# nilsfriess/ParMGMC

Measured on AMD Instinct MI355X. Metric: Gaussian samples/sec on 512^3 3D DMDA (7-pt Laplacian precision, red-black Gibbs sweep = 1 sorgibbs sample), higher is better.
Workload: dtype f64

## Files before the change

parmgmc_amd/csrc/kernels_grid.hip:

```cpp
#include <hip/hip_runtime.h>
#include <cstring>
#include <stdlib.h>
#include "pmg_kernels.h"
#define PMG_RNG_TU grid
#include "pmg_rng.hpp"

namespace {

typedef double d2 __attribute__((ext_vector_type(2)));

__device__ __forceinline__ d2 ld2(const double *p) { return *reinterpret_cast<const d2 *>(p); }

__device__ __forceinline__ d2 ld2_sys(const double *p)
{
  const unsigned long long a = __hip_atomic_load(reinterpret_cast<const unsigned long long *>(p), __ATOMIC_RELAXED, __HIP_MEMORY_SCOPE_SYSTEM);
  const unsigned long long b = __hip_atomic_load(reinterpret_cast<const unsigned long long *>(p) + 1, __ATOMIC_RELAXED, __HIP_MEMORY_SCOPE_SYSTEM);
  d2                       v;
  v.x = __longlong_as_double((long long)a);
  v.y = __longlong_as_double((long long)b);
  return v;
}
__device__ __forceinline__ void st2_sys(double *p, d2 v)
{
  __hip_atomic_store(reinterpret_cast<unsigned long long *>(p), (unsigned long long)__double_as_longlong(v.x), __ATOMIC_RELAXED, __HIP_MEMORY_SCOPE_SYSTEM);
  __hip_atomic_store(reinterpret_cast<unsigned long long *>(p) + 1, (unsigned long long)__double_as_longlong(v.y), __ATOMIC_RELAXED, __HIP_MEMORY_SCOPE_SYSTEM);
}

__device__ __forceinline__ const double *at_bytes(const double *base, uint32_t byte_off) { return reinterpret_cast<const double *>(reinterpret_cast<const char *>(base) + byte_off); }
__device__ __forceinline__ double       *at_bytes(double *base, uint32_t byte_off) { return reinterpret_cast<double *>(reinterpret_cast<char *>(base) + byte_off); }

__device__ __forceinline__ double uniform(double v)
{
  return __hiloint2double(__builtin_amdgcn_readfirstlane(__double2hiint(v)), __builtin_amdgcn_readfirstlane(__double2loint(v)));
}

template <bool PACKED>
__device__ __forceinline__ double table_at(const double (&a)[8], int idx)
{
  if (!PACKED) return uniform(a[idx]);
  double v = a[1];
  v        = idx == 2 ? a[2] : v;
  v        = idx == 3 ? a[3] : v;
  v        = idx == 4 ? a[4] : v;
  v        = idx == 5 ? a[5] : v;
  v        = idx == 6 ? a[6] : v;
  return v;
}

__device__ __forceinline__ void wave_wait_flag(const uint64_t *f, uint64_t v, unsigned *err, unsigned long long *spin_total)
{
  if (threadIdx.x == 0) {
    unsigned long long spins = 0;
    while (__hip_atomic_load(f, __ATOMIC_RELAXED, __HIP_MEMORY_SCOPE_SYSTEM) < v) {
      __builtin_amdgcn_s_sleep(8);
      ++spins;
      if ((spins & 0xFFFFu) == 0 && err && __hip_atomic_load(err, __ATOMIC_RELAXED, __HIP_MEMORY_SCOPE_SYSTEM)) break;
      if (spins > (1ull << 28)) {
        if (err) {
          err[1] = 0x10u;
          err[2] = (unsigned)v;
          err[3] = (unsigned)__hip_atomic_load(f, __ATOMIC_RELAXED, __HIP_MEMORY_SCOPE_SYSTEM);
          __hip_atomic_store(err, 1u, __ATOMIC_RELAXED, __HIP_MEMORY_SCOPE_SYSTEM);
        }
        break;
      }
    }
    if (spins && spin_total) atomicAdd(spin_total, spins);
  }
  __builtin_amdgcn_fence(__ATOMIC_ACQUIRE, "workgroup");
}

template <bool NOISY, bool OMEGA1, bool HALO, bool PACKED>
__device__ __forceinline__ void grid_color_sweep_body(const pmgk_grid_layout &L, const pmgk_grid_op &op, int c, int t, int j, int k, pmg::LogTabEntry *tab, pmg::LogTabEntry tab_entry, const pmgk_grid_halo &halo, const double *__restrict__ b_own, const double *__restrict__ y_other, double *__restrict__ y_own)
{
  const int kg = k + L.kz0;
  bool live = j < L.ny && 2 * t < L.sx && 4 * t + ((c + j + kg) & 1) < L.nx;
  if (NOISY) {
    if (!__builtin_amdgcn_ballot_w64(live)) return;
    t = live ? t : 0;
    if (PACKED) j = live ? j : 0;
  } else if (!live)
    return;
  const int p  = (c + j + kg) & 1;
  const int i0 = 4 * t + p, i1 = i0 + 2;
  const bool v1 = i1 < L.nx;

  const bool    hasS = j > 0, hasN = j < L.ny - 1, hasD = kg > 0, hasU = kg < L.nzg - 1;
  const double  h2 = op.h2;
  const int64_t  rowoff = (int64_t)(k + 1) * L.sp + (int64_t)j * L.sx;
  const uint32_t lo     = 16u * (uint32_t)t;
  const double  *yo_row = y_other + rowoff;
  const int    eo = p ? (2 * t + 2 < L.sx ? 2 : 1) : (t > 0 ? -1 : 0);
  const bool   hasW0 = i0 > 0, hasE0 = i0 < L.nx - 1, hasE1 = i1 < L.nx - 1;
  const int    nyz = PACKED ? (int)hasS + (int)hasN + (int)hasD + (int)hasU : min(j, 1) + min(L.ny - 1 - j, 1) + min(kg, 1) + min(L.nzg - 1 - kg, 1);
  const bool   two0 = hasW0 && hasE0, two1 = hasE1;
  const double idA = table_at<PACKED>(op.idiag, nyz + 1), idB = table_at<PACKED>(op.idiag, nyz + 2);
  const double sqA = NOISY ? table_at<PACKED>(op.sqrtdiag, nyz + 1) : 0.0, sqB = NOISY ? table_at<PACKED>(op.sqrtdiag, nyz + 2) : 0.0;
  double      *out_row = y_own + rowoff;
  d2     Vc = ld2(at_bytes(yo_row, lo));
  double ed = *at_bytes(yo_row, lo + 8u * (uint32_t)eo);
  d2     oS = ld2(at_bytes(yo_row - (hasS ? L.sx : 0), lo));
  d2     oN = ld2(at_bytes(yo_row + (hasN ? L.sx : 0), lo));
  const int64_t inplane = (int64_t)j * L.sx + 2 * t;
  d2      oD = (HALO && k == 0 && halo.glo) ? ld2_sys(halo.glo + inplane) : ld2(at_bytes(yo_row - (hasD ? L.sp : 0), lo));
  d2      oU = (HALO && k == L.nz - 1 && halo.ghi) ? ld2_sys(halo.ghi + inplane) : ld2(at_bytes(yo_row + (hasU ? L.sp : 0), lo));
#ifndef PMG_GRID_NO_NT
  d2     bb = __builtin_nontemporal_load(reinterpret_cast<const d2 *>(at_bytes(b_own + rowoff, lo)));
#else
  d2     bb = ld2(at_bytes(b_own + rowoff, lo));
#endif
  pmg::RngConsts K;
  if (NOISY) {
    __builtin_amdgcn_sched_barrier(0);
    K = pmg::load_sincos_consts();
    __builtin_amdgcn_sched_barrier(0);
  }

  double z0 = 0.0, z1 = 0.0;
  if (NOISY) {
    pmg::normal_pair_fill((uint32_t)t, (uint32_t)(j + (int64_t)L.ny * kg), (uint32_t)op.sweep, ((uint32_t)(op.sweep >> 32) & 0x7fffffffu) | ((uint32_t)c << 31), op.key0, op.key1, tab_entry, tab, (int)threadIdx.x, K, z0, z1);
    asm volatile("" : "+v"(Vc.x), "+v"(Vc.y), "+v"(ed), "+v"(oS.x), "+v"(oS.y), "+v"(oN.x), "+v"(oN.y), "+v"(oD.x), "+v"(oD.y), "+v"(oU.x), "+v"(oU.y), "+v"(bb.x), "+v"(bb.y) : "v"(z0), "v"(z1));
  }
  const double L0 = p ? Vc.x : ed, R0 = p ? Vc.y : Vc.x, L1 = R0, R1 = p ? ed : Vc.y;
  const double idg0 = two0 ? idB : idA, idg1 = two1 ? idB : idA;
  const double hS = hasS ? h2 : 0.0, hN = hasN ? h2 : 0.0, hD = hasD ? h2 : 0.0, hU = hasU ? h2 : 0.0;

  double w0 = bb.x, w1 = bb.y;
  if (NOISY) {
    const double sq0 = two0 ? sqB : sqA, sq1 = two1 ? sqB : sqA;
    w0 = z0 * sq0 + bb.x;
    w1 = z1 * sq1 + bb.y;
  }
  double s0 = w0, s1 = w1;
  s0 = s0 + hD * oD.x;
  s1 = s1 + hD * oD.y;
  s0 = s0 + hS * oS.x;
  s1 = s1 + hS * oS.y;
  s0 = s0 + (hasW0 ? h2 : 0.0) * L0;
  s1 = s1 + h2 * L1;
  s0 = s0 + (hasE0 ? h2 : 0.0) * R0;
  s1 = s1 + (hasE1 ? h2 : 0.0) * R1;
  s0 = s0 + hN * oN.x;
  s1 = s1 + hN * oN.y;
  s0 = s0 + hU * oU.x;
  s1 = s1 + hU * oU.y;

  double r0, r1;
  if (OMEGA1) {
    r0 = idg0 * s0;
    r1 = idg1 * s1;
  } else {
    const d2 yo2 = ld2(at_bytes(out_row, lo));
    r0           = op.one_minus_omega * yo2.x + idg0 * s0;
    r1           = op.one_minus_omega * yo2.y + idg1 * s1;
  }
  const d2 out = {r0, v1 ? r1 : 0.0};
  if (NOISY) {
    asm volatile("" ::"v"(out.x), "v"(out.y), "s"(out_row));
    if (!live) return;
  }
#ifndef PMG_GRID_NO_NT
  __builtin_nontemporal_store(out, reinterpret_cast<d2 *>(at_bytes(out_row, lo)));
#else
  *reinterpret_cast<d2 *>(at_bytes(out_row, lo)) = out;
#endif
  if (HALO) {
    if (k == 0 && halo.plo) st2_sys(halo.plo + inplane, out);
    if (k == L.nz - 1 && halo.phi) st2_sys(halo.phi + inplane, out);
  }
}

template <bool PACKED>
__device__ __forceinline__ void grid_thread_position(int nbx, int bandw, int ty, int &t, int &j)
{
  if (PACKED) {
    const int flat = ((int)blockIdx.x * 4 + ty) * 64 + (int)threadIdx.x;
    j              = flat / nbx;
    t              = flat - j * nbx;
  } else {
    const int bx = bandw > 0 ? (int)(blockIdx.x >> 3) : (int)blockIdx.x;
    const int jl = (int)blockIdx.y * 4 + ty;
    t            = bx * 64 + threadIdx.x;
    j            = bandw > 0 ? (jl < bandw ? (int)(blockIdx.x & 7u) * bandw + jl : 0x40000000) : jl;
  }
}

template <bool NOISY, bool OMEGA1, bool HALO, bool PACKED, bool TAIL>
__global__ __launch_bounds__(256) __attribute__((amdgpu_num_sgpr(96))) void grid_color_sweep_kernel(pmgk_grid_layout L, pmgk_grid_op op, int c, int nbx, int zmain, int bandw, int kbegin, int kstride, int kcount, int tmain, int tailw, pmgk_grid_halo halo, const double *__restrict__ b_own, const double *__restrict__ y_other, double *__restrict__ y_own)
{
  const int ty = __builtin_amdgcn_readfirstlane(threadIdx.y);
  __shared__ pmg::LogTabEntry s_logtab[NOISY ? 4 * PMG_LOGTAB_SIZE : 1];
  pmg::LogTabEntry           *tab = s_logtab + (NOISY ? ty * PMG_LOGTAB_SIZE : 0);
  pmg::LogTabEntry            tab_entry = {0.0, 0.0};
  if (NOISY) {
    const d2 e = ld2(reinterpret_cast<const double *>(pmg::g_logtab + threadIdx.x));
    tab_entry  = {e.x, e.y};
  }
  int                         t, j;
  const int                   zsplit = zmain > 0 ? zmain : kcount;
  if (TAIL && (int)blockIdx.z >= zsplit) {
    const int tb  = (int)blockIdx.x + (int)gridDim.x * ((int)blockIdx.y + (int)gridDim.y * ((int)blockIdx.z - zsplit));
    const bool compact = tailw == 1 && L.nx == 4 * tmain + 1 && (L.sx & 15) != 0;
    const int  slots   = compact ? (L.ny + 1) / 2 : L.ny * tailw;
    const int  per     = (slots + 255) / 256;
    const int  kz = tb / per, part = tb - kz * per;
    if (kz >= kcount) return;
    const int f = (part * 4 + ty) * 64 + (int)threadIdx.x, kt = kbegin + kz * kstride;
    if (compact) {
      j = 2 * f + ((c + kt + L.kz0) & 1);
      t = tmain;
    } else {
      j = f / tailw;
      t = tmain + f - j * tailw;
    }
    grid_color_sweep_body<NOISY, OMEGA1, false, true>(L, op, c, t, j, kt, tab, tab_entry, halo, b_own, y_other, y_own);
    return;
  }
  grid_thread_position<PACKED>(nbx, bandw, ty, t, j);

  int k = kbegin + (int)blockIdx.z * kstride;
  if (!HALO && !PACKED && zmain > 0) {
    const int xcd = (int)(blockIdx.x & 7u), extra = max(xcd - (8 - (L.ny - 8 * bandw)), 0);
    const int first = xcd * bandw + extra, nl = bandw + (xcd >= 8 - (L.ny - 8 * bandw) ? 1 : 0);
    const int w     = ((int)blockIdx.y + (int)gridDim.y * (int)blockIdx.z) * 4 + ty;
    if (nl <= 0) return;
    const int kz = w / nl;
    if (kz >= kcount) return;
    t = (int)(blockIdx.x >> 3) * 64 + (int)threadIdx.x;
    j = first + (w - kz * nl);
    k = kbegin + kz * kstride;
  }
  if (HALO && halo.full) {
    const int z = (int)blockIdx.z;
    k           = z == 0 ? 0 : (z == 1 ? L.nz - 1 : z - 1);
    const bool face_lo = k == 0, face_hi = k == L.nz - 1;
    if (face_lo && halo.wlo) wave_wait_flag(halo.wlo, halo.wval, halo.err, halo.spins);
    if (face_hi && halo.whi) wave_wait_flag(halo.whi, halo.wval, halo.err, halo.spins);
    grid_color_sweep_body<NOISY, OMEGA1, HALO, PACKED>(L, op, c, t, j, k, tab, tab_entry, halo, b_own, y_other, y_own);
    if (face_lo || face_hi) {
      asm volatile("s_waitcnt vmcnt(0)" ::: "memory");
      __builtin_amdgcn_fence(__ATOMIC_RELEASE, "workgroup");
      __syncthreads();
      if (threadIdx.x == 0 && threadIdx.y == 0) {
        const unsigned nface  = L.nz > 1 ? 2u : 1u;
        const unsigned expect = gridDim.x * gridDim.y * nface;
        if (atomicAdd(halo.counter, 1u) == expect - 1u) {
          *halo.counter = 0;
          if (halo.slo) __hip_atomic_store(halo.slo, halo.sval, __ATOMIC_RELAXED, __HIP_MEMORY_SCOPE_SYSTEM);
          if (halo.shi) __hip_atomic_store(halo.shi, halo.sval, __ATOMIC_RELAXED, __HIP_MEMORY_SCOPE_SYSTEM);
        }
      }
    }
    return;
  }
  grid_color_sweep_body<NOISY, OMEGA1, HALO, PACKED>(L, op, c, t, j, k, tab, tab_entry, halo, b_own, y_other, y_own);
}

__global__ void grid_to_cvec_kernel(pmgk_grid_layout L, const double *__restrict__ nat, double *__restrict__ cv)
{
  const int i = blockIdx.x * blockDim.x + threadIdx.x;
  const int j = blockIdx.y * blockDim.y + threadIdx.y;
  const int k = blockIdx.z;
  if (i >= L.nx || j >= L.ny) return;
  const int c = (i + j + k + L.kz0) & 1;
  cv[(int64_t)c * L.cs + (int64_t)(k + 1) * L.sp + (int64_t)j * L.sx + (i >> 1)] = nat[i + (int64_t)L.nx * (j + (int64_t)L.ny * k)];
}

__global__ void grid_from_cvec_kernel(pmgk_grid_layout L, const double *__restrict__ cv, double *__restrict__ nat)
{
  const int i = blockIdx.x * blockDim.x + threadIdx.x;
  const int j = blockIdx.y * blockDim.y + threadIdx.y;
  const int k = blockIdx.z;
  if (i >= L.nx || j >= L.ny) return;
  const int c = (i + j + k + L.kz0) & 1;
  nat[i + (int64_t)L.nx * (j + (int64_t)L.ny * k)] = cv[(int64_t)c * L.cs + (int64_t)(k + 1) * L.sp + (int64_t)j * L.sx + (i >> 1)];
}

struct residual_consts {
  double a, dA, dB, aS, aN, aD, aU;
};

__device__ __forceinline__ d2 residual_pair(const residual_consts &K, bool hasW0, bool hasE0, bool hasE1, bool v1, d2 oD, d2 oS, d2 oN, d2 oU, double L0, double R0, double L1, double R1, d2 yy, d2 bb)
{
  const double dg0 = (hasW0 && hasE0) ? K.dB : K.dA, dg1 = hasE1 ? K.dB : K.dA;
  double       s0 = 0.0, s1 = 0.0;
  s0 = s0 + K.aD * oD.x;
  s1 = s1 + K.aD * oD.y;
  s0 = s0 + K.aS * oS.x;
  s1 = s1 + K.aS * oS.y;
  s0 = s0 + (hasW0 ? K.a : 0.0) * L0;
  s1 = s1 + K.a * L1;
  s0 = s0 + dg0 * yy.x;
  s1 = s1 + dg1 * yy.y;
  s0 = s0 + (hasE0 ? K.a : 0.0) * R0;
  s1 = s1 + (hasE1 ? K.a : 0.0) * R1;
  s0 = s0 + K.aN * oN.x;
  s1 = s1 + K.aN * oN.y;
  s0 = s0 + K.aU * oU.x;
  s1 = s1 + K.aU * oU.y;
  const d2 out = {bb.x - s0, v1 ? bb.y - s1 : 0.0};
  return out;
}

template <bool PACKED>
__device__ __forceinline__ void grid_residual_values(const pmgk_grid_layout &L, const pmgk_grid_op &op, int t, int j, int k, const double *__restrict__ b, const double *__restrict__ y, int64_t &offa, int64_t &offb, d2 &outA, d2 &outB)
{
  const int      kg   = k + L.kz0;
  const int      ca   = (j + kg) & 1;
  const bool     hasS = j > 0, hasN = j < L.ny - 1, hasD = kg > 0, hasU = kg < L.nzg - 1;
  const int64_t  rowoff = (int64_t)(k + 1) * L.sp + (int64_t)j * L.sx;
  const uint32_t lo     = 16u * (uint32_t)t;
  offa = (int64_t)ca * L.cs + rowoff;
  offb = (int64_t)(1 - ca) * L.cs + rowoff;
  const double  *ya = y + offa, *yb = y + offb;
  const int64_t  dS = hasS ? L.sx : 0, dN = hasN ? L.sx : 0, dD = hasD ? L.sp : 0, dU = hasU ? L.sp : 0;
  const d2       Ya = ld2(at_bytes(ya, lo)), Yb = ld2(at_bytes(yb, lo));
  const double   edA = *at_bytes(yb, lo - (t > 0 ? 8u : 0u));
  const double   edB = *at_bytes(ya, lo + (2 * t + 2 < L.sx ? 16u : 8u));
  const int      nyz = (int)hasS + (int)hasN + (int)hasD + (int)hasU;
  residual_consts K;
  K.a  = -op.h2;
  K.dA = table_at<PACKED>(op.diag, nyz + 1);
  K.dB = table_at<PACKED>(op.diag, nyz + 2);
  K.aS = hasS ? K.a : 0.0;
  K.aN = hasN ? K.a : 0.0;
  K.aD = hasD ? K.a : 0.0;
  K.aU = hasU ? K.a : 0.0;
  const int i0 = 4 * t;
  outA = residual_pair(K, i0 > 0, i0 < L.nx - 1, i0 + 2 < L.nx - 1, i0 + 2 < L.nx, ld2(at_bytes(yb - dD, lo)), ld2(at_bytes(yb - dS, lo)), ld2(at_bytes(yb + dN, lo)), ld2(at_bytes(yb + dU, lo)), edA, Yb.x, Yb.x, Yb.y, Ya, ld2(at_bytes(b + offa, lo)));
  outB = d2{0.0, 0.0};
  if (i0 + 1 < L.nx)
    outB = residual_pair(K, true, i0 + 1 < L.nx - 1, i0 + 3 < L.nx - 1, i0 + 3 < L.nx, ld2(at_bytes(ya - dD, lo)), ld2(at_bytes(ya - dS, lo)), ld2(at_bytes(ya + dN, lo)), ld2(at_bytes(ya + dU, lo)), Ya.x, Ya.y, Ya.y, edB, Yb, ld2(at_bytes(b + offb, lo)));
}

template <bool PACKED>
__device__ __forceinline__ void grid_residual_body(const pmgk_grid_layout &L, const pmgk_grid_op &op, int t, int j, int k, const double *__restrict__ b, const double *__restrict__ y, double *__restrict__ r)
{
  if (j >= L.ny || 2 * t >= L.sx || 4 * t >= L.nx) return;
  int64_t offa, offb;
  d2      outA, outB;
  grid_residual_values<PACKED>(L, op, t, j, k, b, y, offa, offb, outA, outB);
  const uint32_t lo = 16u * (uint32_t)t;
  *reinterpret_cast<d2 *>(at_bytes(r + offa, lo)) = outA;
  if (4 * t + 1 < L.nx) *reinterpret_cast<d2 *>(at_bytes(r + offb, lo)) = outB;
}

__device__ __forceinline__ double lane_prev_d(double v)
{
  return __hiloint2double(__builtin_amdgcn_update_dpp(0, __double2hiint(v), 0x138, 0xf, 0xf, false), __builtin_amdgcn_update_dpp(0, __double2loint(v), 0x138, 0xf, 0xf, false));
}
__device__ __forceinline__ double lane_next_d(double v)
{
  return __hiloint2double(__builtin_amdgcn_update_dpp(0, __double2hiint(v), 0x130, 0xf, 0xf, false), __builtin_amdgcn_update_dpp(0, __double2loint(v), 0x130, 0xf, 0xf, false));
}

struct rr_acc {
  double s0, s1;
};
struct rr_thread {
  int      t, J0;
  uint32_t lo;
  bool     left, right0, right1;
  bool     eW0, eE0, eE1, eV1;
  bool     oE0, oE1, oV1, ovalid;
};

__device__ __forceinline__ void rr_add(rr_acc &a, double wyz, const rr_thread &T, double Lf, const d2 &E, const d2 &O)
{
  const double h = 0.5 * wyz;
  a.s0 = a.s0 + (T.left ? h : 0.0) * Lf;
  a.s0 = a.s0 + wyz * E.x;
  a.s0 = a.s0 + (T.right0 ? h : 0.0) * O.x;
  a.s1 = a.s1 + h * O.x;
  a.s1 = a.s1 + wyz * E.y;
  a.s1 = a.s1 + (T.right1 ? h : 0.0) * O.y;
}

struct rr_line {
  d2 ev, od;
};

struct rr_planes {
  const double *v, *lo2, *hi2;
  int           kz0, nz;
  uint32_t      sp8, cs8;
};
struct rr_plane {
  const double *p;
  uint32_t      base, cst;
};
__device__ __forceinline__ rr_plane rr_plane_of(const rr_planes &P, int g)
{
  const int kl = g - P.kz0;
  rr_plane  r;
  if (kl >= -1 && kl <= P.nz) {
    r.p    = P.v;
    r.base = (uint32_t)(kl + 1) * P.sp8;
    r.cst  = P.cs8;
  } else {
    r.p    = kl < 0 ? P.lo2 : P.hi2;
    r.base = 0;
    r.cst  = P.sp8;
  }
  return r;
}

__device__ __forceinline__ rr_line rr_load_line(const rr_plane &pl, uint32_t line, int parity)
{
  const uint32_t c = parity ? pl.cst : 0u;
  rr_line        r;
  r.ev = ld2(at_bytes(pl.p, pl.base + line + c));
  r.od = ld2(at_bytes(pl.p, pl.base + line + (pl.cst - c)));
  return r;
}

template <bool SYNC>
__global__ __launch_bounds__(256) void grid_residual_restrict_kernel(pmgk_grid_layout L, pmgk_grid_op op, pmgk_st27_dims C, int tplE, int wpp, int kc, int nchunks, const double *__restrict__ b, const double *__restrict__ y, const double *__restrict__ ylo2, const double *__restrict__ yhi2, double *__restrict__ bc)
{
  const int xcd = (int)blockIdx.x & 7, q = (int)blockIdx.x >> 3, per = (int)gridDim.x >> 3;
  const int gw  = __builtin_amdgcn_readfirstlane((xcd * per + q) * 4 + (int)(threadIdx.x >> 6));
  const int wppb = SYNC ? (wpp + 3) / 4 * 4 : wpp;
  const int zc = gw / wppb, wv = gw - zc * wppb;
  if (zc >= nchunks) return;
  const int  lane = threadIdx.x & 63, nslots = C.ny * tplE;
  const int  fu = 62 * wv + lane - 1, f = min(max(fu, 0), nslots - 1);
  const bool store = lane >= 1 && lane <= 62 && fu < nslots;
  rr_thread  T;
  const int  Jc = f / tplE;
  T.t      = f - Jc * tplE;
  T.J0     = Jc;
  T.lo     = 16u * (uint32_t)T.t;
  const int i0 = 4 * T.t, I0 = 2 * T.t;
  T.left   = I0 > 0;
  T.right0 = i0 + 1 < L.nx;
  T.right1 = i0 + 3 < L.nx;
  T.eW0    = i0 > 0;
  T.eE0    = i0 < L.nx - 1;
// ... 67 lines not shown
#endif
      const rr_line &S = i == 0 ? hS : Cv[i > 0 ? i - 1 : 0], &N = i == 2 ? hN : Cv[i < 2 ? i + 1 : 2];
      const bool     hasS = jc > 0, hasN = jc < jmax, inner = hasS && hasN;
      residual_consts Kc;
      Kc.a  = ma;
      Kc.dA = inner ? dg3 : dg2;
      Kc.dB = inner ? dg4 : dg3;
      Kc.aS = hasS ? ma : 0.0;
      Kc.aN = hasN ? ma : 0.0;
      Kc.aD = hasD ? ma : 0.0;
      Kc.aU = hasU ? ma : 0.0;
      const double edA = lane_prev_d(Cv[i].od.y), edB = lane_next_d(Cv[i].ev.x);
      const d2     E = residual_pair(Kc, T.eW0, T.eE0, T.eE1, T.eV1, Dv[i].ev, S.ev, N.ev, Uv[i].ev, edA, Cv[i].od.x, Cv[i].od.x, Cv[i].od.y, Cv[i].ev, bb.ev);
      d2           O = residual_pair(Kc, true, T.oE0, T.oE1, T.oV1, Dv[i].od, S.od, N.od, Uv[i].od, Cv[i].ev.x, Cv[i].ev.y, Cv[i].ev.y, edB, Cv[i].od, bb.od);
      if (!T.ovalid) O = d2{0.0, 0.0};
      const double Lf = lane_prev_d(O.y);
      const double w  = ((unsigned)j < (unsigned)L.ny) ? (i == 1 ? wz : 0.5 * wz) : 0.0;
      rr_add(a, w, T, Lf, E, O);
      if (odd) rr_add(n, w, T, Lf, E, O);
    }
    if (odd) {
      if (k > 2 * K0 - 1) {
        if (store) {
          out[0] = a.s0;
          if (I0 + 1 < C.nx) out[1] = a.s1;
        }
        out += cplane;
      }
      a = n;
      n = rr_acc{0.0, 0.0};
    }
#pragma unroll
    for (int i = 0; i < 3; ++i) {
      Dv[i] = Cv[i];
      Cv[i] = Uv[i];
    }
    hS = hSu;
    hN = hNu;
  }
  if (2 * K1 - 1 > klast && store) {
    out[0] = a.s0;
    if (I0 + 1 < C.nx) out[1] = a.s1;
  }
}

template <bool PACKED, bool TAIL>
__global__ __launch_bounds__(256) void grid_residual_kernel(pmgk_grid_layout L, pmgk_grid_op op, int bandw, int tplE, int tmain, int tailw, const double *__restrict__ b, const double *__restrict__ y, double *__restrict__ r)
{
  const int ty = __builtin_amdgcn_readfirstlane(threadIdx.y);
  if (TAIL && (int)blockIdx.z >= L.nz) {
    const int tb  = (int)blockIdx.x + (int)gridDim.x * ((int)blockIdx.y + (int)gridDim.y * ((int)blockIdx.z - L.nz));
    const int per = (L.ny * tailw + 255) / 256;
    const int kz = tb / per, part = tb - kz * per;
    if (kz >= L.nz) return;
    const int f = (part * 4 + ty) * 64 + (int)threadIdx.x, j = f / tailw;
    grid_residual_body<true>(L, op, tmain + f - j * tailw, j, kz, b, y, r);
    return;
  }
  int t, j;
  grid_thread_position<PACKED>(tplE, bandw, ty, t, j);
  grid_residual_body<PACKED>(L, op, t, j, (int)blockIdx.z, b, y, r);
}

inline int launch_status() { return hipGetLastError() == hipSuccess ? 0 : 1; }

}

static inline int grid_threads_per_line(const pmgk_grid_layout *L) { return ((L->nx + 1) / 2 + 1) / 2; }
static inline bool grid_use_packed(const pmgk_grid_layout *L)
{
  static int env = -1;
  if (env < 0) {
    const char *e = getenv("PMG_GRID_PACKED");
    env           = e ? atoi(e) : 2;
  }
  if (env != 2) return env == 1;
  const int tplE = grid_threads_per_line(L), lanes = (L->sx / 2 + 63) / 64 * 64;
  return 2 * lanes >= 3 * tplE;
}

struct grid_mapping {
  bool packed, tail;
  int  nbx, nby, bandw, tmain, tailw, ztail, zmain;
  dim3 grid;
};

static grid_mapping grid_choose_mapping(const pmgk_grid_layout *L, int kcount, bool allow_tail, bool allow_flat = false)
{
  static int banded_env = -1, tail_env = -1, flat_env = -1;
  if (banded_env < 0) {
    const char *e = getenv("PMG_GRID_BANDED");
    banded_env    = e ? atoi(e) : 1;
    e             = getenv("PMG_GRID_TAIL");
    tail_env      = e ? atoi(e) : 1;
    e             = getenv("PMG_GRID_FLAT");
    flat_env      = e ? atoi(e) : 1;
  }
  grid_mapping M;
  const int    tpl = L->sx / 2, tplE = grid_threads_per_line(L);
  M.nby   = (L->ny + 3) / 4;
  M.tmain = tplE / 64 * 64;
  M.tailw = tplE - M.tmain;
  M.tail   = allow_tail && tail_env && M.tmain > 0 && M.tailw > 0 && M.tailw <= 8;
  M.packed = !M.tail && grid_use_packed(L);
  M.nbx    = M.packed ? tplE : (M.tail ? M.tmain / 64 : (tpl + 63) / 64);
  M.bandw = (!M.packed && banded_env && M.nby >= 16) ? (L->ny + 7) / 8 : 0;
  M.ztail = 0;
  M.zmain = 0;
  if (M.packed) M.grid = dim3((unsigned)(((int64_t)L->ny * tplE + 255) / 256), 1, kcount);
  else {
    const unsigned gx = M.bandw > 0 ? 8 * M.nbx : M.nbx, gy = M.bandw > 0 ? (M.bandw + 3) / 4 : M.nby;
    if (allow_flat && flat_env && M.bandw > 0 && ((M.bandw & 3) || 8 * M.bandw != L->ny)) {
      M.bandw           = L->ny / 8;
      const int maxband = M.bandw + (L->ny > 8 * M.bandw ? 1 : 0);
      M.zmain           = (int)(((int64_t)maxband * kcount + 4 * gy - 1) / (4 * gy));
    }
    const int zlayers = M.zmain > 0 ? M.zmain : kcount;
    if (M.tail) {
      const int64_t nblocks = (int64_t)kcount * (((int64_t)L->ny * M.tailw + 255) / 256);
      M.ztail               = (int)((nblocks + (int64_t)gx * gy - 1) / ((int64_t)gx * gy));
    }
    M.grid = dim3(gx, gy, zlayers + M.ztail);
  }
  if (!M.tail) M.tmain = M.tailw = 0;
  return M;
}

template <bool NOISY, bool OMEGA1, bool HALO>
static void launch_sweep(const grid_mapping &M, dim3 block, hipStream_t s, const pmgk_grid_layout &L, const pmgk_grid_op &op, int color, int kbegin, int kstride, int kcount, const pmgk_grid_halo &h, const double *bo, const double *yo, double *ys)
{
  if (M.packed) hipLaunchKernelGGL((grid_color_sweep_kernel<NOISY, OMEGA1, HALO, true, false>), M.grid, block, 0, s, L, op, color, M.nbx, 0, M.bandw, kbegin, kstride, kcount, 0, 0, h, bo, yo, ys);
  else if (!HALO && M.tail) hipLaunchKernelGGL((grid_color_sweep_kernel<NOISY, OMEGA1, false, false, true>), M.grid, block, 0, s, L, op, color, M.nbx, M.zmain, M.bandw, kbegin, kstride, kcount, M.tmain, M.tailw, h, bo, yo, ys);
  else hipLaunchKernelGGL((grid_color_sweep_kernel<NOISY, OMEGA1, HALO, false, false>), M.grid, block, 0, s, L, op, color, M.nbx, HALO ? 0 : M.zmain, M.bandw, kbegin, kstride, kcount, 0, 0, h, bo, yo, ys);
}

extern "C" int pmgk_grid_color_sweep(const pmgk_grid_layout *L, const pmgk_grid_op *op, int color, int kbegin, int kcount, int kstride, const pmgk_grid_halo *halo, const double *b, double *y, void *stream)
{
  if (kcount <= 0) return 0;
  const grid_mapping M = grid_choose_mapping(L, kcount, !halo, !halo);
  const dim3         block(64, 4, 1);
  hipStream_t   s  = (hipStream_t)stream;
  const double *bo = b + (int64_t)color * L->cs, *yo = y + (int64_t)(1 - color) * L->cs;
  double       *ys = y + (int64_t)color * L->cs;
  pmgk_grid_halo h0;
  memset(&h0, 0, sizeof h0);
  if (halo) {
    if (op->noisy) {
      if (op->omega_is_one) launch_sweep<true, true, true>(M, block, s, *L, *op, color, kbegin, kstride, kcount, *halo, bo, yo, ys);
      else launch_sweep<true, false, true>(M, block, s, *L, *op, color, kbegin, kstride, kcount, *halo, bo, yo, ys);
    } else {
      if (op->omega_is_one) launch_sweep<false, true, true>(M, block, s, *L, *op, color, kbegin, kstride, kcount, *halo, bo, yo, ys);
      else launch_sweep<false, false, true>(M, block, s, *L, *op, color, kbegin, kstride, kcount, *halo, bo, yo, ys);
    }
  } else if (op->noisy) {
    if (op->omega_is_one) launch_sweep<true, true, false>(M, block, s, *L, *op, color, kbegin, kstride, kcount, h0, bo, yo, ys);
    else launch_sweep<true, false, false>(M, block, s, *L, *op, color, kbegin, kstride, kcount, h0, bo, yo, ys);
  } else {
    if (op->omega_is_one) launch_sweep<false, true, false>(M, block, s, *L, *op, color, kbegin, kstride, kcount, h0, bo, yo, ys);
    else launch_sweep<false, false, false>(M, block, s, *L, *op, color, kbegin, kstride, kcount, h0, bo, yo, ys);
  }
  return launch_status();
}

extern "C" int pmgk_grid_residual(const pmgk_grid_layout *L, const pmgk_grid_op *op, const double *b, const double *y, double *r, void *stream)
{
  if (L->nz <= 0) return 0;
  const grid_mapping M = grid_choose_mapping(L, L->nz, true);
  const dim3         block(64, 4, 1);
  const int          tplE = grid_threads_per_line(L);
  if (M.packed) hipLaunchKernelGGL((grid_residual_kernel<true, false>), M.grid, block, 0, (hipStream_t)stream, *L, *op, M.bandw, tplE, 0, 0, b, y, r);
  else if (M.tail) hipLaunchKernelGGL((grid_residual_kernel<false, true>), M.grid, block, 0, (hipStream_t)stream, *L, *op, M.bandw, tplE, M.tmain, M.tailw, b, y, r);
  else hipLaunchKernelGGL((grid_residual_kernel<false, false>), M.grid, block, 0, (hipStream_t)stream, *L, *op, M.bandw, tplE, 0, 0, b, y, r);
  return launch_status();
}

extern "C" int pmgk_grid_residual_restrict_applies(const pmgk_grid_layout *L, const pmgk_st27_dims *C, int have_lo2, int have_hi2)
{
  static const int off  = getenv("PMG_GRID_FUSED_RR") ? !atoi(getenv("PMG_GRID_FUSED_RR")) : 0;
  const int        tplE = grid_threads_per_line(L);
  const bool       slab = L->kz0 != 0 || L->nz != L->nzg;
  if (off || C->nz <= 0) return 0;
  if (!slab && (C->kz0 != 0 || C->nz != C->nzg)) return 0;
  if (slab && ((L->kz0 > 0 && !have_lo2) || (L->kz0 + L->nz < L->nzg && !have_hi2) || L->nz < 2)) return 0;
  if (L->nx < 3 || L->ny < 3 || L->nzg < 3 || !(L->nx & 1) || !(L->ny & 1) || !(L->nzg & 1)) return 0;
  if (C->nx != (L->nx + 1) / 2 || C->ny != (L->ny + 1) / 2 || C->nzg != (L->nzg + 1) / 2) return 0;
  if (tplE != (C->nx + 1) / 2 || (int64_t)C->ny * tplE >= ((int64_t)1 << 30)) return 0;
  if (2 * (int64_t)L->cs * 8 >= ((int64_t)1 << 32)) return 0;
  if (slab && (2 * C->kz0 < L->kz0 || 2 * (C->kz0 + C->nz - 1) >= L->kz0 + L->nz)) return 0;
  return 1;
}

extern "C" int pmgk_grid_residual_restrict(const pmgk_grid_layout *L, const pmgk_grid_op *op, const pmgk_st27_dims *C, const double *b, const double *y, const double *ylo2, const double *yhi2, double *bc, void *stream)
{
  static const int kc_env = getenv("PMG_GRID_RR_CHUNK") ? atoi(getenv("PMG_GRID_RR_CHUNK")) : 0;
  if (!pmgk_grid_residual_restrict_applies(L, C, ylo2 != nullptr, yhi2 != nullptr)) return -1;
  const int     tplE = grid_threads_per_line(L);
  static const int sync_knob = getenv("PMG_GRID_RR_SYNC") ? atoi(getenv("PMG_GRID_RR_SYNC")) : -1;
  const int        sync_env  = sync_knob >= 0 ? sync_knob : ((int64_t)L->nx * L->ny * L->nz >= 8000000);
  const int     wpp = (int)(((int64_t)C->ny * tplE + 61) / 62);
  int           kc  = kc_env > 0 ? kc_env : 8;
  while (kc_env <= 0 && kc > 2 && (int64_t)wpp * ((C->nz + kc - 1) / kc) < 2048) kc >>= 1;
  const int     nchunks = (C->nz + kc - 1) / kc;
  if (sync_env) {
    const int64_t nblocks = (int64_t)((wpp + 3) / 4) * nchunks;
    hipLaunchKernelGGL(grid_residual_restrict_kernel<true>, dim3((unsigned)((nblocks + 7) / 8 * 8)), dim3(256), 0, (hipStream_t)stream, *L, *op, *C, tplE, wpp, kc, nchunks, b, y, ylo2, yhi2, bc);
  } else {
    const int64_t nblocks = ((int64_t)wpp * nchunks + 3) / 4;
    hipLaunchKernelGGL(grid_residual_restrict_kernel<false>, dim3((unsigned)((nblocks + 7) / 8 * 8)), dim3(256), 0, (hipStream_t)stream, *L, *op, *C, tplE, wpp, kc, nchunks, b, y, ylo2, yhi2, bc);
  }
  return launch_status();
}

extern "C" int pmgk_grid_to_cvec(const pmgk_grid_layout *L, const double *nat, double *cvec, void *stream)
{
  const dim3 block(64, 4, 1);
  const dim3 grid((L->nx + 63) / 64, (L->ny + 3) / 4, L->nz);
  hipLaunchKernelGGL(grid_to_cvec_kernel, grid, block, 0, (hipStream_t)stream, *L, nat, cvec);
  return launch_status();
}

extern "C" int pmgk_grid_from_cvec(const pmgk_grid_layout *L, const double *cvec, double *nat, void *stream)
{
  const dim3 block(64, 4, 1);
  const dim3 grid((L->nx + 63) / 64, (L->ny + 3) / 4, L->nz);
  hipLaunchKernelGGL(grid_from_cvec_kernel, grid, block, 0, (hipStream_t)stream, *L, cvec, nat);
  return launch_status();
}
```

parmgmc_amd/csrc/pmg_kernels.h:

```cpp
#ifndef PMG_KERNELS_H
#define PMG_KERNELS_H
#include <stdint.h>
#ifdef __cplusplus
extern "C" {
#endif

typedef struct {
  int32_t nx, ny, nz;
  int32_t kz0, nzg;
  int32_t sx;
  int64_t sp;
  int64_t cs;
} pmgk_grid_layout;

typedef struct {
  double   h2;
  double   one_minus_omega;
  double   idiag[8];
  double   sqrtdiag[8];
  double   diag[8];
  uint32_t key0, key1;
  uint64_t sweep;
  int32_t  noisy;
  int32_t  omega_is_one;
} pmgk_grid_op;

typedef struct {
  const double *glo, *ghi;
  double       *plo, *phi;
  int32_t       full;
  const uint64_t *wlo, *whi;
  uint64_t       wval;
  uint64_t      *slo, *shi;
  uint64_t       sval;
  unsigned      *counter, *err;
  unsigned long long *spins;
} pmgk_grid_halo;
int pmgk_grid_color_sweep(const pmgk_grid_layout *L, const pmgk_grid_op *op, int color, int kbegin, int kcount, int kstride, const pmgk_grid_halo *halo, const double *b_cvec, double *y_cvec, void *stream);
int pmgk_grid_to_cvec(const pmgk_grid_layout *L, const double *nat, double *cvec, void *stream);
int pmgk_grid_from_cvec(const pmgk_grid_layout *L, const double *cvec, double *nat, void *stream);
int pmgk_grid_residual(const pmgk_grid_layout *L, const pmgk_grid_op *op, const double *b_cvec, const double *y_cvec, double *r_cvec, void *stream);

typedef struct {
  int32_t        n;
  int32_t        ld;
  int32_t        nslices;
  const int64_t *soff;
  const int32_t *swidth;
  const double  *vals;
  const int32_t *cols;
  const double  *idiag;
  const double  *sqrtdiag;
  const double  *diag;
  const int32_t *orig;
  int64_t        noise_row0;
} pmgk_sell;

int pmgk_sell_color_sweep(const pmgk_sell *S, int slice0, int nsl, double omega, int noisy, uint64_t seed, uint64_t sweep, const double *b, double *y, void *stream);
int pmgk_sell_residual(const pmgk_sell *S, const double *b, const double *y, double *r, void *stream);
int pmgk_permute_in(int32_t ld, const int32_t *orig, const double *nat, double *perm, void *stream);
int pmgk_permute_out(int32_t ld, const int32_t *orig, const double *perm, double *nat, void *stream);

int pmgk_csr_spmv(int32_t nrows, const int32_t *rowptr, const int32_t *colidx, const double *vals, double alpha, const double *x, double beta, double *y, void *stream);
int pmgk_csr_spmv_rows(int32_t nrows, const int32_t *rowpos, const int32_t *rowptr, const int32_t *colidx, const double *vals, const double *x, double *y, int accumulate, double *zero, void *stream);
int pmgk_potrf_inverse(int32_t npad, double *A_colmajor, double *W_colmajor, double *T_scratch, double *Dinv_scratch, int *info_dev, void *stream);
int pmgk_pack_rowmajor(int32_t n, const double *in_colmajor, int64_t ld, int transpose, double *out_rowmajor, void *stream);
typedef struct {
  int32_t       nx, ny, nz;
  int32_t       kz0, nzg;
  const double *coef, *idiag, *sqrtdiag;
} pmgk_st27;
typedef struct {
  int32_t nx, ny, nz, kz0, nzg;
} pmgk_st27_dims;
int pmgk_st27_sweep(const pmgk_st27 *S, int backward, double omega, int noisy, uint64_t seed, uint64_t sweep, const double *b, double *y, void *stream);
int pmgk_st27_sweep_phase(const pmgk_st27 *S, int backward, int phase, double omega, int noisy, uint64_t seed, uint64_t sweep, const double *b, double *y, void *stream);
int pmgk_st27_residual(const pmgk_st27 *S, const double *b, const double *y, double *r, void *stream);
int pmgk_st27_sweep_pp(const pmgk_st27 *S, int backward, double omega, int noisy, uint64_t seed, uint64_t sweep, const double *b, const double *y_in, double *y_out, void *stream);
int pmgk_st27_sweep_pp_phase(const pmgk_st27 *S, int backward, int phase, double omega, int noisy, uint64_t seed, uint64_t sweep, const double *b, const double *y_in, double *y_out, void *stream);
int pmgk_st27_residual_pair(const pmgk_st27 *S, const double *b, const double *y, double *r, void *stream);
int pmgk_st27_restrict(const pmgk_st27_dims *F, const pmgk_st27_dims *C, const double *r, double *bc, void *stream);
int pmgk_st27_prolong_add(const pmgk_st27_dims *F, const pmgk_st27_dims *C, int kbegin, int kcount, const double *ec, double *x, void *stream);
int pmgk_q1_restrict(const pmgk_grid_layout *L, const pmgk_st27_dims *C, const int32_t *cpos, const double *r_cvec, double *bc, void *stream);
int pmgk_grid_residual_restrict_applies(const pmgk_grid_layout *L, const pmgk_st27_dims *C, int have_lo2, int have_hi2);
int pmgk_grid_residual_restrict(const pmgk_grid_layout *L, const pmgk_grid_op *op, const pmgk_st27_dims *C, const double *b_cvec, const double *y_cvec, const double *ylo2, const double *yhi2, double *bc, void *stream);
int pmgk_q1_prolong_add(const pmgk_grid_layout *L, const pmgk_st27_dims *C, const int32_t *cpos, int kbegin, int kcount, int only_color, const double *ec, double *x_cvec, void *stream);
int pmgk_tri_gemv(int32_t n, int upper, const double *M, const double *x, const double *add, double *out, void *stream);
int pmgk_lrc_nblocks(int64_t n);
int pmgk_lrc_rows_per_block(void);
int pmgk_lrc_rows_nblocks(int64_t ns);
int pmgk_lrc_btx(int64_t n, int k, const double *M, int64_t ld, const double *y, double *partial, const double *scale, double *out, void *stream);
int pmgk_lrc_axpy_cols(int64_t n, int k, const double *M, int64_t ld, const double *coef, double sign, const double *in, double *out, void *stream);
int pmgk_lrc_gemm_small(int64_t n, int k, const double *Cm, int64_t ld, const double *Sb, double *Bb, void *stream);
int pmgk_lrc_mark_rows(int64_t n, int k, const double *A0, const double *A1, const double *A2, int64_t ld, unsigned char *mask, void *stream);
int pmgk_lrc_gather_rows(int64_t ns, int k, const double *M, int64_t ld, const int64_t *rows, double *Mc, void *stream);
int pmgk_lrc_reduce_axpy_rows(int64_t ns, int k, const double *Mc, const int64_t *rows, int nb, const double *partial, const double *scale, double sign, double *v, double *save, void *stream);
int pmgk_lrc_reduce_axpy_btx_rows(int64_t ns, int k, const double *Mb, const int64_t *rows, const double *partial_in, double sign, double *v, const double *Mc, double *partial_out, void *stream);
int pmgk_lrc_btx_rows(int64_t ns, int k, const double *Mc, const int64_t *rows, const double *y, double *partial, const double *scale, double *out, const double *save, double *w, void *stream);
int pmgk_lrc_axpy_rows(int64_t ns, int k, const double *Mc, const int64_t *rows, const double *coef, double sign, double *v, double *save, void *stream);
int pmgk_lrc_scatter_rows(int64_t ns, const int64_t *rows, const double *save, double *v, void *stream);
int pmgk_lrc_axpy_restore_rows(int64_t ns, int k, const double *Mc, const int64_t *rows, const double *coef, double sign, double *v, const double *save, double *w, void *stream);
int pmgk_lrc_rhs_rows(int64_t ns, int k, const double *Mc, const int64_t *rows, const double *sqrtS, uint64_t seed, uint64_t sweep, double *b, double *save, void *stream);
int pmgk_lrc_btx_axpy_small(int64_t ns1, int k, const double *M1, const int64_t *rows1, const double *y, const double *scale, double *wk, int64_t ns2, const double *M2, const int64_t *rows2, double sign, double *v, const double *save, double *w, void *stream);
int pmgk_axpy(int64_t n, double alpha, const double *x, double *y, void *stream);
int pmgk_fill_zero(double *p, int64_t n, void *stream);
int pmgk_stream_triad(int64_t n, const double *a, const double *b, double *c, void *stream);
int pmgk_sum_rows(int nrows, int count, const double *in, double *out, void *stream);
#define PMGK_XCH_MAXSEG 8
typedef struct {
  int           nseg;
  const double *src[PMGK_XCH_MAXSEG];
  double       *dst[PMGK_XCH_MAXSEG];
  int64_t       n[PMGK_XCH_MAXSEG];
  uint64_t     *flag[4];
  uint64_t      value[4];
} pmgk_xch_args;
int pmgk_xch_push(const pmgk_xch_args *a, unsigned *counter, void *stream);
int pmgk_xch_push_dbg(const pmgk_xch_args *a, unsigned *counter, unsigned *dbg, void *stream);
int pmgk_allgather_push(int nranks, int me, const double *src, int64_t n, double *const *dst_dev, int64_t dst_off, uint64_t *const *flag_dev, uint64_t value, unsigned *counter, void *stream);
int pmgk_allgather_wait(int nranks, int me, const uint64_t *myflags, uint64_t value, unsigned *err, void *stream);
int pmgk_xch_pull(const pmgk_xch_args *a, unsigned *err, void *stream);
// ... 39 lines not shown
```

Baseline: 1663.

## Get neighbour edge values via DPP lane shifts; use reciprocal multiply in flat mapping

In the non-packed sweep path, the per-thread scalar load of the adjacent east/west value is replaced by a DPP cross-lane shift of the already-loaded d2 vector. Only wave-edge lanes use a single uniform load. This cuts one gathered global load per thread, but inactive lanes must now stay alive to feed their neighbours. Separately, the flat banded mapping replaces an integer division with a precomputed reciprocal multiply that is validated on the host, and two helper entry points are added for checking geometry.

```diff
diff --git a/parmgmc_amd/csrc/kernels_grid.hip b/parmgmc_amd/csrc/kernels_grid.hip
--- a/parmgmc_amd/csrc/kernels_grid.hip
+++ b/parmgmc_amd/csrc/kernels_grid.hip
@@ -32,6 +32,15 @@
 __device__ __forceinline__ double uniform(double v)
 {
   return __hiloint2double(__builtin_amdgcn_readfirstlane(__double2hiint(v)), __builtin_amdgcn_readfirstlane(__double2loint(v)));
+}
+
+__device__ __forceinline__ double lane_prev_d(double v)
+{
+  return __hiloint2double(__builtin_amdgcn_update_dpp(0, __double2hiint(v), 0x138, 0xf, 0xf, false), __builtin_amdgcn_update_dpp(0, __double2loint(v), 0x138, 0xf, 0xf, false));
+}
+__device__ __forceinline__ double lane_next_d(double v)
+{
+  return __hiloint2double(__builtin_amdgcn_update_dpp(0, __double2hiint(v), 0x130, 0xf, 0xf, false), __builtin_amdgcn_update_dpp(0, __double2loint(v), 0x130, 0xf, 0xf, false));
 }
 
 template <bool PACKED>
@@ -75,9 +84,15 @@
 {
   const int kg = k + L.kz0;
   bool live = j < L.ny && 2 * t < L.sx && 4 * t + ((c + j + kg) & 1) < L.nx;
-  if (NOISY) {
+#ifndef PMG_GRID_ED_LOAD
+  constexpr bool LANE_ED = !PACKED;
+#else
+  constexpr bool LANE_ED = false;
+#endif
+  const int t0 = LANE_ED ? t - (int)threadIdx.x : 0;
+  if (NOISY || LANE_ED) {
     if (!__builtin_amdgcn_ballot_w64(live)) return;
-    t = live ? t : 0;
+    t = (LANE_ED ? 2 * t < L.sx : live) ? t : 0;
     if (PACKED) j = live ? j : 0;
   } else if (!live)
     return;
@@ -98,7 +113,9 @@
   const double sqA = NOISY ? table_at<PACKED>(op.sqrtdiag, nyz + 1) : 0.0, sqB = NOISY ? table_at<PACKED>(op.sqrtdiag, nyz + 2) : 0.0;
   double      *out_row = y_own + rowoff;
   d2     Vc = ld2(at_bytes(yo_row, lo));
-  double ed = *at_bytes(yo_row, lo + 8u * (uint32_t)eo);
+  double ed = 0.0, es = 0.0;
+  if (!LANE_ED) ed = *at_bytes(yo_row, lo + 8u * (uint32_t)eo);
+  else es = yo_row[min(max(2 * t0 - 1 + 129 * p, 0), L.sx - 1)];
   d2     oS = ld2(at_bytes(yo_row - (hasS ? L.sx : 0), lo));
   d2     oN = ld2(at_bytes(yo_row + (hasN ? L.sx : 0), lo));
   const int64_t inplane = (int64_t)j * L.sx + 2 * t;
@@ -119,7 +136,20 @@
   double z0 = 0.0, z1 = 0.0;
   if (NOISY) {
     pmg::normal_pair_fill((uint32_t)t, (uint32_t)(j + (int64_t)L.ny * kg), (uint32_t)op.sweep, ((uint32_t)(op.sweep >> 32) & 0x7fffffffu) | ((uint32_t)c << 31), op.key0, op.key1, tab_entry, tab, (int)threadIdx.x, K, z0, z1);
-    asm volatile("" : "+v"(Vc.x), "+v"(Vc.y), "+v"(ed), "+v"(oS.x), "+v"(oS.y), "+v"(oN.x), "+v"(oN.y), "+v"(oD.x), "+v"(oD.y), "+v"(oU.x), "+v"(oU.y), "+v"(bb.x), "+v"(bb.y) : "v"(z0), "v"(z1));
+    if (!LANE_ED) asm volatile("" : "+v"(ed));
+    else asm volatile("" : "+s"(es));
+    asm volatile("" : "+v"(Vc.x), "+v"(Vc.y), "+v"(oS.x), "+v"(oS.y), "+v"(oN.x), "+v"(oN.y), "+v"(oD.x), "+v"(oD.y), "+v"(oU.x), "+v"(oU.y), "+v"(bb.x), "+v"(bb.y) : "v"(z0), "v"(z1));
+  }
+  if (LANE_ED) {
+    const int lane = (int)threadIdx.x;
+    if (p) {
+      ed = lane_next_d(Vc.x);
+      ed = lane == 63 ? es : ed;
+      ed = 2 * t + 2 < L.sx ? ed : Vc.y;
+    } else {
+      ed = lane_prev_d(Vc.y);
+      ed = lane == 0 ? es : ed;
+    }
   }
   const double L0 = p ? Vc.x : ed, R0 = p ? Vc.y : Vc.x, L1 = R0, R1 = p ? ed : Vc.y;
   const double idg0 = two0 ? idB : idA, idg1 = two1 ? idB : idA;
@@ -155,8 +185,8 @@
     r1           = op.one_minus_omega * yo2.y + idg1 * s1;
   }
   const d2 out = {r0, v1 ? r1 : 0.0};
-  if (NOISY) {
-    asm volatile("" ::"v"(out.x), "v"(out.y), "s"(out_row));
+  if (NOISY || LANE_ED) {
+    if (NOISY) asm volatile("" ::"v"(out.x), "v"(out.y), "s"(out_row));
     if (!live) return;
   }
 #ifndef PMG_GRID_NO_NT
@@ -185,8 +215,17 @@
   }
 }
 
+__host__ __device__ __forceinline__ void grid_flat_position(int ny, int bandw, uint32_t rcp0, uint32_t rcp1, int xcd, int w, int &kz, int &j)
+{
+  const int  nshort   = 8 - (ny - 8 * bandw);
+  const bool longband = xcd >= nshort;
+  const int  first = xcd * bandw + (longband ? xcd - nshort : 0), nl = bandw + (longband ? 1 : 0);
+  kz = (int)(uint32_t)(((uint64_t)(uint32_t)w * (longband ? rcp1 : rcp0)) >> 32);
+  j  = first + (w - kz * nl);
+}
+
 template <bool NOISY, bool OMEGA1, bool HALO, bool PACKED, bool TAIL>
-__global__ __launch_bounds__(256) __attribute__((amdgpu_num_sgpr(96))) void grid_color_sweep_kernel(pmgk_grid_layout L, pmgk_grid_op op, int c, int nbx, int zmain, int bandw, int kbegin, int kstride, int kcount, int tmain, int tailw, pmgk_grid_halo halo, const double *__restrict__ b_own, const double *__restrict__ y_other, double *__restrict__ y_own)
+__global__ __launch_bounds__(256) __attribute__((amdgpu_num_sgpr(96))) void grid_color_sweep_kernel(pmgk_grid_layout L, pmgk_grid_op op, int c, int nbx, int zmain, int bandw, int kbegin, int kstride, int kcount, int tmain, int tailw, uint32_t rcp0, uint32_t rcp1, pmgk_grid_halo halo, const double *__restrict__ b_own, const double *__restrict__ y_other, double *__restrict__ y_own)
 {
   const int ty = __builtin_amdgcn_readfirstlane(threadIdx.y);
   __shared__ pmg::LogTabEntry s_logtab[NOISY ? 4 * PMG_LOGTAB_SIZE : 1];
@@ -220,14 +259,11 @@
 
   int k = kbegin + (int)blockIdx.z * kstride;
   if (!HALO && !PACKED && zmain > 0) {
-    const int xcd = (int)(blockIdx.x & 7u), extra = max(xcd - (8 - (L.ny - 8 * bandw)), 0);
-    const int first = xcd * bandw + extra, nl = bandw + (xcd >= 8 - (L.ny - 8 * bandw) ? 1 : 0);
-    const int w     = ((int)blockIdx.y + (int)gridDim.y * (int)blockIdx.z) * 4 + ty;
-    if (nl <= 0) return;
-    const int kz = w / nl;
+    const int w = ((int)blockIdx.y + (int)gridDim.y * (int)blockIdx.z) * 4 + ty;
+    int       kz;
+    grid_flat_position(L.ny, bandw, rcp0, rcp1, (int)(blockIdx.x & 7u), w, kz, j);
     if (kz >= kcount) return;
     t = (int)(blockIdx.x >> 3) * 64 + (int)threadIdx.x;
-    j = first + (w - kz * nl);
     k = kbegin + kz * kstride;
   }
   if (HALO && halo.full) {
@@ -345,14 +381,6 @@
   if (4 * t + 1 < L.nx) *reinterpret_cast<d2 *>(at_bytes(r + offb, lo)) = outB;
 }
 
-__device__ __forceinline__ double lane_prev_d(double v)
-{
-  return __hiloint2double(__builtin_amdgcn_update_dpp(0, __double2hiint(v), 0x138, 0xf, 0xf, false), __builtin_amdgcn_update_dpp(0, __double2loint(v), 0x138, 0xf, 0xf, false));
-}
-__device__ __forceinline__ double lane_next_d(double v)
-{
-  return __hiloint2double(__builtin_amdgcn_update_dpp(0, __double2hiint(v), 0x130, 0xf, 0xf, false), __builtin_amdgcn_update_dpp(0, __double2loint(v), 0x130, 0xf, 0xf, false));
-}
 
 struct rr_acc {
   double s0, s1;
@@ -586,8 +614,21 @@
 struct grid_mapping {
   bool packed, tail;
   int  nbx, nby, bandw, tmain, tailw, ztail, zmain;
+  uint32_t rcp0, rcp1;
   dim3 grid;
 };
+
+static bool grid_flat_reciprocals(int bandw, int64_t wcount, uint32_t &rcp0, uint32_t &rcp1)
+{
+  if (bandw < 2 || wcount <= 0 || wcount > (int64_t)1 << 31) return false;
+  uint32_t *r[2] = {&rcp0, &rcp1};
+  for (int i = 0; i < 2; ++i) {
+    const uint64_t nl = (uint64_t)bandw + i, m = ((uint64_t)1 << 32) / nl + 1, e = m * nl - ((uint64_t)1 << 32);
+    if (m >> 32 || (uint64_t)(wcount - 1) * e >= (uint64_t)1 << 32) return false;
+    *r[i] = (uint32_t)m;
+  }
+  return true;
+}
 
 static grid_mapping grid_choose_mapping(const pmgk_grid_layout *L, int kcount, bool allow_tail, bool allow_flat = false)
 {
@@ -611,13 +652,18 @@
   M.bandw = (!M.packed && banded_env && M.nby >= 16) ? (L->ny + 7) / 8 : 0;
   M.ztail = 0;
   M.zmain = 0;
+  M.rcp0 = M.rcp1 = 0;
   if (M.packed) M.grid = dim3((unsigned)(((int64_t)L->ny * tplE + 255) / 256), 1, kcount);
   else {
     const unsigned gx = M.bandw > 0 ? 8 * M.nbx : M.nbx, gy = M.bandw > 0 ? (M.bandw + 3) / 4 : M.nby;
     if (allow_flat && flat_env && M.bandw > 0 && ((M.bandw & 3) || 8 * M.bandw != L->ny)) {
-      M.bandw           = L->ny / 8;
-      const int maxband = M.bandw + (L->ny > 8 * M.bandw ? 1 : 0);
-      M.zmain           = (int)(((int64_t)maxband * kcount + 4 * gy - 1) / (4 * gy));
+      const int     fbandw  = L->ny / 8;
+      const int     maxband = fbandw + (L->ny > 8 * fbandw ? 1 : 0);
+      const int64_t zmain   = ((int64_t)maxband * kcount + 4 * gy - 1) / (4 * gy);
+      if (grid_flat_reciprocals(fbandw, 4 * (int64_t)gy * zmain, M.rcp0, M.rcp1)) {
+        M.bandw = fbandw;
+        M.zmain = (int)zmain;
+      }
     }
     const int zlayers = M.zmain > 0 ? M.zmain : kcount;
     if (M.tail) {
@@ -633,9 +679,9 @@
 template <bool NOISY, bool OMEGA1, bool HALO>
 static void launch_sweep(const grid_mapping &M, dim3 block, hipStream_t s, const pmgk_grid_layout &L, const pmgk_grid_op &op, int color, int kbegin, int kstride, int kcount, const pmgk_grid_halo &h, const double *bo, const double *yo, double *ys)
 {
-  if (M.packed) hipLaunchKernelGGL((grid_color_sweep_kernel<NOISY, OMEGA1, HALO, true, false>), M.grid, block, 0, s, L, op, color, M.nbx, 0, M.bandw, kbegin, kstride, kcount, 0, 0, h, bo, yo, ys);
-  else if (!HALO && M.tail) hipLaunchKernelGGL((grid_color_sweep_kernel<NOISY, OMEGA1, false, false, true>), M.grid, block, 0, s, L, op, color, M.nbx, M.zmain, M.bandw, kbegin, kstride, kcount, M.tmain, M.tailw, h, bo, yo, ys);
-  else hipLaunchKernelGGL((grid_color_sweep_kernel<NOISY, OMEGA1, HALO, false, false>), M.grid, block, 0, s, L, op, color, M.nbx, HALO ? 0 : M.zmain, M.bandw, kbegin, kstride, kcount, 0, 0, h, bo, yo, ys);
+  if (M.packed) hipLaunchKernelGGL((grid_color_sweep_kernel<NOISY, OMEGA1, HALO, true, false>), M.grid, block, 0, s, L, op, color, M.nbx, 0, M.bandw, kbegin, kstride, kcount, 0, 0, 0u, 0u, h, bo, yo, ys);
+  else if (!HALO && M.tail) hipLaunchKernelGGL((grid_color_sweep_kernel<NOISY, OMEGA1, false, false, true>), M.grid, block, 0, s, L, op, color, M.nbx, M.zmain, M.bandw, kbegin, kstride, kcount, M.tmain, M.tailw, M.rcp0, M.rcp1, h, bo, yo, ys);
+  else hipLaunchKernelGGL((grid_color_sweep_kernel<NOISY, OMEGA1, HALO, false, false>), M.grid, block, 0, s, L, op, color, M.nbx, HALO ? 0 : M.zmain, M.bandw, kbegin, kstride, kcount, 0, 0, M.rcp0, M.rcp1, h, bo, yo, ys);
 }
 
 extern "C" int pmgk_grid_color_sweep(const pmgk_grid_layout *L, const pmgk_grid_op *op, int color, int kbegin, int kcount, int kstride, const pmgk_grid_halo *halo, const double *b, double *y, void *stream)
@@ -666,6 +712,31 @@
   return launch_status();
 }
 
+extern "C" int pmgk_grid_sweep_geometry(const pmgk_grid_layout *L, int kcount, int32_t out[9])
+{
+  const grid_mapping M = grid_choose_mapping(L, kcount, true, true);
+  const int32_t      v[9] = {M.packed, M.tail, M.bandw, M.zmain, (int32_t)M.grid.x, (int32_t)M.grid.y, (int32_t)M.grid.z, (int32_t)M.rcp0, (int32_t)M.rcp1};
+  memcpy(out, v, sizeof v);
+  return 0;
+}
+
+extern "C" int64_t pmgk_grid_flat_check(const pmgk_grid_layout *L, int kcount)
+{
+  const grid_mapping M = grid_choose_mapping(L, kcount, true, true);
+  if (M.zmain <= 0) return 0;
+  int64_t bad = 0;
+  for (int xcd = 0; xcd < 8; ++xcd) {
+    const int nshort = 8 - (L->ny - 8 * M.bandw), nl = M.bandw + (xcd >= nshort ? 1 : 0);
+    const int first  = xcd * M.bandw + (xcd >= nshort ? xcd - nshort : 0);
+    for (int64_t w = 0; w < 4 * (int64_t)M.grid.y * M.zmain; ++w) {
+      int kz, j;
+      grid_flat_position(L->ny, M.bandw, M.rcp0, M.rcp1, xcd, (int)w, kz, j);
+      bad += kz != (int)(w / nl) || j != first + (int)(w % nl);
+    }
+  }
+  return bad;
+}
+
 extern "C" int pmgk_grid_residual(const pmgk_grid_layout *L, const pmgk_grid_op *op, const double *b, const double *y, double *r, void *stream)
 {
   if (L->nz <= 0) return 0;
diff --git a/parmgmc_amd/csrc/pmg_kernels.h b/parmgmc_amd/csrc/pmg_kernels.h
--- a/parmgmc_amd/csrc/pmg_kernels.h
+++ b/parmgmc_amd/csrc/pmg_kernels.h
@@ -37,6 +37,8 @@
   unsigned long long *spins;
 } pmgk_grid_halo;
 int pmgk_grid_color_sweep(const pmgk_grid_layout *L, const pmgk_grid_op *op, int color, int kbegin, int kcount, int kstride, const pmgk_grid_halo *halo, const double *b_cvec, double *y_cvec, void *stream);
+int     pmgk_grid_sweep_geometry(const pmgk_grid_layout *L, int kcount, int32_t out[9]);
+int64_t pmgk_grid_flat_check(const pmgk_grid_layout *L, int kcount);
 int pmgk_grid_to_cvec(const pmgk_grid_layout *L, const double *nat, double *cvec, void *stream);
 int pmgk_grid_from_cvec(const pmgk_grid_layout *L, const double *cvec, double *nat, void *stream);
 int pmgk_grid_residual(const pmgk_grid_layout *L, const pmgk_grid_op *op, const double *b_cvec, const double *y_cvec, double *r_cvec, void *stream);
```

Result: no change. 1649 (-0.8%).
